# algoterranean/3dgan

Hardware: AMD Instinct MI355X
Metric: images/sec (whole node), CIFAR-10 IWGAN bs=512 (higher is better)
Workload: dtype bf16; 1 GPU; --model iwgan --dataset cifar(32x32x3 synthetic) --batch_size 512/GPU --latent_size 200 --optimizer adam --lr 1e-4 --beta1 0.5 --beta2 0.9 --n_disc_train 5; one step = 5 D + 1 G optimizer steps on 6 fresh batches; global_batch=512, parallelism=dp1, ranks_seen=1

## Files before the change

3dgan_amd/csrc/tdg_igemm.hip:

```cpp
#include <stdlib.h>

#include "tdg_igemm.h"
#include "tdg_wgrad_patch.h"
#include <type_traits>

#define OOB_OFFSET 0xFFFFFF00u

#ifdef TDG_STAMPS
#define TDG_STAMP(var)                                                                            \
  do {                                                                                            \
    __builtin_amdgcn_sched_barrier(0);                                                            \
    asm volatile("s_memtime %0\n\ts_waitcnt lgkmcnt(0)" : "=s"(var)::"memory");                  \
    __builtin_amdgcn_sched_barrier(0);                                                            \
  } while (0)
#else
#define TDG_STAMP(var) do { } while (0)
#endif

template <int I, int N, class F>
__device__ __forceinline__ void static_for(F&& f) {
  if constexpr (I < N) {
    f(IntC<I>{});
    static_for<I + 1, N>(f);
  }
// ... 965 lines not shown
    if (mmode != TDG_MASK_NONE) {
#pragma unroll
      for (int e = 0; e < 8; ++e) v[e] = (bf16_t)((float)v[e] * ((float)mv[it][e] > 0.f ? 1.f : mlow));
      if (args.col_partial) *reinterpret_cast<bf16x8*>(sE + row * PE + cc * 16) = v;
    }
    if (n + 8 <= N) {
      *reinterpret_cast<bf16x8*>(out + p + n) = v;
    } else {
      *reinterpret_cast<bf16x4*>(out + p + n) = bf16x4{v[0], v[1], v[2], v[3]};
    }
  }
  if (args.col_partial) {
    constexpr int G = NTHR / BN > 0 ? NTHR / BN : 1;
    float* sRed = reinterpret_cast<float*>(smem + BM * PE + BM * 8);
    __syncthreads();
    const int mlim = args.col_images > 0 ? min(M, args.col_images * cl.GH * cl.GW * (cl.nbh * cl.nbw > 1 ? cl.nbh * cl.nbw : 1)) : M;
    const int rows_valid = max(0, min(BM, mlim - m0));
    const int col = tid % BN, grp = tid / BN;
    const bool bnm = args.col_mode == TDG_COL_BN;
    if (grp < G) {
      const float piv = bnm ? sBias[col] : 0.f;
      float s0 = 0.f, s1 = 0.f;
      for (int r = grp; r < rows_valid; r += G) {
        const float v = (float)*reinterpret_cast<const bf16_t*>(sE + r * PE + col * 2) - piv;
        s0 += v;
        s1 += v * v;
      }
      sRed[(grp * 2 + 0) * BN + col] = s0;
      sRed[(grp * 2 + 1) * BN + col] = s1;
    }
    __syncthreads();
    if (tid < BN && n0 + tid < N) {
      float t0 = 0.f, t1 = 0.f;
#pragma unroll
      for (int g = 0; g < G; ++g) { t0 += sRed[(g * 2 + 0) * BN + tid]; t1 += sRed[(g * 2 + 1) * BN + tid]; }
      float* pr = args.col_partial + (size_t)(blockIdx.z * args.ntiles_m_max + tile_m) * 2 * N;
      pr[n0 + tid] = t0;
      pr[N + n0 + tid] = t1;
    }
  }
}

#ifndef PT_VBLOCK
#define PT_VBLOCK 32
#endif
#ifndef PT_LA
#define PT_LA 3
#endif
template <int TM, int TN, int ABL, int t>
__device__ __forceinline__ void patch_half0(f32x4 (&acc)[TM][TN], const bf16x8 (&fa0)[TM], bf16x8 (&fa1)[TM], bf16x8 (&fb)[2 * TN + PT_LA],
                                            const char* smem, const int (&a1)[TM], const char* pB, int coff0, int coff1) {
  if constexpr (t < TN) {
    constexpr int t2 = t + PT_LA, ks2 = t2 / TN, j2 = t2 - ks2 * TN;
    if constexpr (ABL != 1) fb[t2] = *reinterpret_cast<const bf16x8*>(pB + j2 * 16 * IG_BKB + (ks2 ? coff1 : coff0));
    else fb[t2] = fb[t2 & 1];
    if constexpr (t < TM && ABL != 2) fa1[t] = pt_lds_frag(a1[t]);
#pragma unroll
    for (int i = 0; i < TM; ++i) Mma<bf16_t>::run(acc[i][t], fb[t], fa0[i]);
    __builtin_amdgcn_sched_group_barrier(0x100, 1 + (t < TM ? 1 : 0), 0);
    __builtin_amdgcn_sched_group_barrier(0x008, TM, 0);
    patch_half0<TM, TN, ABL, t + 1>(acc, fa0, fa1, fb, smem, a1, pB, coff0, coff1);
  }
}
template <int TM, int TN, int ABL, int t>
__device__ __forceinline__ void patch_half1(f32x4 (&acc)[TM][TN], bf16x8 (&fa0)[TM], const bf16x8 (&fa1)[TM], bf16x8 (&fb)[2 * TN + PT_LA],
                                            const char* smem, const int (&a0n)[TM], const char* pB, const char* pBn, int coff0, int coff1) {
  constexpr int NT = 2 * TN;
  if constexpr (t < NT) {
    constexpr int j = t - TN, t2 = t + PT_LA;
    if constexpr (ABL == 1) fb[t2] = fb[t2 & 1];
    else if constexpr (t2 < NT) fb[t2] = *reinterpret_cast<const bf16x8*>(pB + (t2 - TN) * 16 * IG_BKB + coff1);
    else fb[t2] = *reinterpret_cast<const bf16x8*>(pBn + (t2 - NT) * 16 * IG_BKB + coff0);
    constexpr int a_lo = TN > TM ? (j >= 1 && j <= TM ? j - 1 : 0) : (j * TM) / TN;
    constexpr int a_hi = TN > TM ? (j >= 1 && j <= TM ? j : 0) : ((j + 1) * TM) / TN;
    if constexpr (ABL != 2) static_for<a_lo, a_hi>([&](auto i_c) { constexpr int i = decltype(i_c)::value; fa0[i] = pt_lds_frag(a0n[i]); });
#pragma unroll
    for (int i = 0; i < TM; ++i) Mma<bf16_t>::run(acc[i][j], fb[t], fa1[i]);
    __builtin_amdgcn_sched_group_barrier(0x100, 1 + (a_hi - a_lo), 0);
    __builtin_amdgcn_sched_group_barrier(0x008, TM, 0);
    patch_half1<TM, TN, ABL, t + 1>(acc, fa0, fa1, fb, smem, a0n, pB, pBn, coff0, coff1);
  }
}

template <int BM, int BN, int ABL, int CK = PT_CK, int PIECES = PT_PIECES>
__global__ void __launch_bounds__(512, 2) igemm_fwd_patch_kernel(const IgArgs args) {
  using T = bf16_t;
  constexpr int NTHR = 512, CW = 4, LW = 4;
  constexpr int PATCHB = PIECES * 1024, PPW = (PIECES + LW - 1) / LW, PPW0 = (PPW + 1) / 2;
  constexpr int WMR = BM / CW, TM = WMR / 16, TN = BN / 16;
  constexpr int BNL = 2 * ((BN / 16 + 1) / 2) * 16;
  constexpr int NIB = BNL / 8, NBJ = (NIB + LW - 1) / LW;
  constexpr int STAGE = BNL * IG_BKB, NS = 3;
  static_assert(PIECES % LW == 0, "patch pieces are dealt evenly to the loader waves");
  static_assert(BM % (16 * CW) == 0 && BN % 16 == 0 && BN / 16 >= BM / (16 * CW), "tile config: the K step hands out one A fragment per column tile");
  constexpr int OFF_ZERO = 0, OFF_RING = PT_ZEROB, OFF_PATCH = OFF_RING + NS * STAGE, OFF_TAB = OFF_PATCH + PT_NPB * PATCHB;
  typedef __attribute__((address_space(3))) void* lds_ptr_t;

  extern __shared__ __attribute__((aligned(16))) char smem[];
  const IgClass& cl = args.cls[blockIdx.z];
  const int tid = threadIdx.x;
  const int bid = xcd_remap(blockIdx.x, gridDim.x);
  const int tile_m = bid / args.ntiles_n;
  const int tile_n = bid - tile_m * args.ntiles_n;
  const int M = cl.M;
  const int nsteps = cl.nsteps;
  int* sTab = reinterpret_cast<int*>(smem + OFF_TAB);
  float* sBias = reinterpret_cast<float*>(smem + OFF_TAB + nsteps * 8 * 8);
  if (tile_m * BM >= M) {
    if (args.col_partial && tid < BN) {
      const int n = args.n_begin + tile_n * BN + tid;
      float* pr = args.col_partial + (size_t)(blockIdx.z * args.ntiles_m_max + tile_m) * 2 * args.N;
      if (n < args.N) { pr[n] = 0.f; pr[args.N + n] = 0.f; }
    }
    return;
  }
  const int m0 = tile_m * BM, n0 = args.n_begin + tile_n * BN;
  const int wave = __builtin_amdgcn_readfirstlane(tid >> 6), lane = tid & 63;
  const bool is_mma = wave < CW;
  const int ntaps = cl.ntaps, G = cl.ngroups, QH = cl.QH, QW = cl.QW;
  const int GHW = cl.GH * cl.GW;
  const int SLC = ntaps * CK;
  const int halo = cl.halo;
  const int P = args.nslices * G;

  unsigned long long ph0 = 0, ph1 = 0, php = 0, t0 = 0, t1 = 0, t2 = 0, s_issue = 0, s_mma = 0, s_sync = 0;
  unsigned long long q0 = 0, q1 = 0, q2 = 0, q3 = 0;
  TDG_STAMP(ph0);
  const float bias_v = (tid < BNL && args.bias && n0 + tid < args.N) ? args.bias[n0 + tid] : 0.f;
  if (tid < PT_ZEROB / 4) reinterpret_cast<int*>(smem + OFF_ZERO)[tid] = 0;
  if ((unsigned)(size_t)(lds_ptr_t)smem != 0u) __builtin_trap();
  TDG_STAMP(q0);
  int tapvec = 0;
  if (is_mma) {
    int tw[IG_MAX_TAPS / 2], g_t0[4], g_ph[4], g_pw[4];
    const int sgs = args.sigma - 1;
#pragma unroll
    for (int k = 0; k < IG_MAX_TAPS / 2; ++k) tw[k] = reinterpret_cast<const int*>(cl.tap)[k];
#pragma unroll
    for (int k = 0; k < 4; ++k) { g_t0[k] = cl.grp[k].t0; g_ph[k] = cl.grp[k].ph; g_pw[k] = cl.grp[k].pw; }
    {
      const int t = lane & (IG_MAX_TAPS - 1);
      int w = tw[0];
#pragma unroll
      for (int k = 1; k < IG_MAX_TAPS / 2; ++k) w = (t >> 1) == k ? tw[k] : w;
      int gi = 0, ph = g_ph[0], pw = g_pw[0];
#pragma unroll
      for (int k = 1; k < 4; ++k) {
        const bool in = k < G && t >= g_t0[k];
        gi = in ? k : gi; ph = in ? g_ph[k] : ph; pw = in ? g_pw[k] : pw;
      }
      const int pk = (t & 1) ? (w >> 16) : w;
      const int dhq = (tap_dh(pk) - ph) >> sgs, dwq = (tap_dw(pk) - pw) >> sgs;
      tapvec = gi | ((dhq + 8) << 4) | ((dwq + 8) << 8);
    }
    TDG_STAMP(q1);
    for (int g0 = 0; g0 < nsteps * 8; g0 += 64 * CW) {
      const int g = g0 + tid;
      const unsigned u = fd_div((unsigned)g, args.fd_ck);
      const int j = g - (int)u * CK;
      const unsigned sl = fd_div(u, cl.fd_nt);
      const int t = (int)(u - sl * (unsigned)ntaps);
      const int tv = __builtin_amdgcn_ds_bpermute((t & 31) << 2, tapvec);
      int w0 = 0, w1 = 31;
      if ((int)sl < args.nslices) {
        const int gi = tv & 15, dhq = ((tv >> 4) & 15) - 8, dwq = ((tv >> 8) & 15) - 8;
        const int p = (int)sl * G + gi;
        const int buf = p - (p / PT_NPB) * PT_NPB;
        w0 = OFF_PATCH + buf * PATCHB + (dhq * QW + dwq) * PT_PIXB + j * 16;
        w1 = t;
      }
      if (g < nsteps * 8) {
        sTab[2 * g] = w0;
        sTab[2 * g + 1] = w1;
      }
    }
// ... 3 lines not shown
  TDG_STAMP(q3);

  const int r16 = lane & 15, q = lane >> 4;
  f32x4 acc[TM][TN];
#pragma unroll
  for (int i = 0; i < TM; ++i)
#pragma unroll
    for (int j = 0; j < TN; ++j) acc[i][j] = f32x4{0.f, 0.f, 0.f, 0.f};

  if (!is_mma) {
    const int lwave = wave - CW;
    const int par = lwave & 1, wh = lwave >> 1, rsub = lane >> 3;
    const __amdgpu_buffer_rsrc_t rA = make_rsrc(args.src, args.src_bytes);
    const __amdgpu_buffer_rsrc_t rB = make_rsrc(static_cast<const char*>(args.wpack) + cl.w_off_bytes, args.w_bytes - cl.w_off_bytes);
    const int lch = (lane & 7) ^ ((4 * par + (rsub >> 1)) & 7);
    unsigned b_row[NBJ];
    int b_lds[NBJ];
#pragma unroll
    for (int j = 0; j < NBJ; ++j) {
      const int I = 2 * (wh + (LW / 2) * j) + par;
      const int n = n0 + 8 * I + rsub;
      const bool useful = 8 * I < BN;
      b_row[j] = (useful && n < args.N) ? ((unsigned)n * (unsigned)cl.Kp + (unsigned)(lch * 8)) * 2u : OOB_OFFSET;
      b_lds[j] = (I < NIB ? I : NIB - 1) * 1024;
    }
    auto b_pieces = [&](int step) {
      const int st = step - (step / NS) * NS;
      char* stage = smem + OFF_RING + st * STAGE;
      const unsigned kb = step < nsteps ? (unsigned)step * IG_BKB : OOB_OFFSET;
#pragma unroll
      for (int j = 0; j < NBJ; ++j) {
        const unsigned off = (b_row[j] == OOB_OFFSET || kb == OOB_OFFSET) ? OOB_OFFSET : b_row[j] + kb;
        __builtin_amdgcn_raw_ptr_buffer_load_lds(rB, (lds_ptr_t)(stage + b_lds[j]), 16, off, 0, 0, 0);
      }
    };
    struct Ph { int sl, gi, buf; };
    auto ph_next = [&](Ph& x) {
      if (++x.gi == G) { x.gi = 0; ++x.sl; }
      x.buf = x.buf == PT_NPB - 1 ? 0 : x.buf + 1;
    };
    auto ph_end_chunk = [&](const Ph& x) { return x.sl * SLC + (cl.grp[x.gi].t0 + cl.grp[x.gi].nt) * CK; };
    auto ph_delta = [&](const Ph& x) { return (unsigned)(((cl.grp[x.gi].ph * args.SW + cl.grp[x.gi].pw) * args.Cs + x.sl * CK * 8) * 2); };
    asm volatile("s_waitcnt lgkmcnt(0)" ::: "memory");
    b_pieces(0);
    const int IPT = BM / GHW;
    const int nimg = M / GHW;
    const int nblk = cl.nbh * cl.nbw;
    const int LH = args.SH / args.sigma, LW_ = args.SW / args.sigma;
    unsigned a_src[PPW];
#pragma unroll
    for (int ps = 0; ps < PPW; ++ps) {
      const int c = (ps * LW + lwave) * 64 + lane;
      const int pl = c / PT_CK, j = c - pl * PT_CK;
      const unsigned il = fd_div((unsigned)pl, cl.fd_qhw);
      const int rem = pl - (int)il * QH * QW;
      const int qh = (int)fd_div((unsigned)rem, cl.fd_qw), qw = rem - qh * QW;
      const int blk = tile_m * IPT + (int)il;
      bool ok = (int)il < IPT && blk < nimg && j < CK;
      int img = blk, lh = qh, lw = qw;
      if (nblk > 1) {
        img = blk / nblk;
        const int br = blk - img * nblk, bi = br / cl.nbw, bj = br - bi * cl.nbw;
        lh = bi * cl.GH - halo + qh;
        lw = bj * cl.GW - halo + qw;
        ok = ok && (unsigned)lh < (unsigned)LH && (unsigned)lw < (unsigned)LW_;
      }
      a_src[ps] = ok ? (unsigned)((((img * args.SH + args.sigma * lh) * args.SW + args.sigma * lw) * args.Cs + j * 8) * 2) : OOB_OFFSET;
    }
    auto a_piece = [&](const Ph& x, unsigned delta, auto ps_c) {
      constexpr int ps = decltype(ps_c)::value;
      const unsigned off = a_src[ps] == OOB_OFFSET ? OOB_OFFSET : a_src[ps] + delta;
      __builtin_amdgcn_raw_ptr_buffer_load_lds(rA, (lds_ptr_t)(smem + OFF_PATCH + x.buf * PATCHB + (ps * LW + lwave) * 1024), 16, off, 0, 0, 0);
    };
    auto a_pieces = [&](const Ph& x, unsigned delta, auto lo_c, auto hi_c) {
      static_for<decltype(lo_c)::value, decltype(hi_c)::value>([&](auto ps_c) { a_piece(x, delta, ps_c); });
    };
    Ph pn{0, 0, 0};
    {
      const unsigned dl0 = ph_delta(pn);
      a_pieces(pn, dl0, IntC<0>{}, IntC<PPW>{});
      ph_next(pn);
    }
    b_pieces(1);
    TDG_STAMP(t0);
    s_mma = t0 - ph0;
    asm volatile("s_waitcnt vmcnt(%0)" ::"n"(NBJ) : "memory");
    __builtin_amdgcn_s_barrier();
    TDG_STAMP(php);
    Ph pf{0, 0, 0};
    int left = P - 1;
    int ready = P > PT_NPB ? (ph_end_chunk(pf) - 1) / 8 + 1 : (1 << 30);
    if (ready < PT_NPB - 1) ready = PT_NPB - 1;
    unsigned dl = left > 0 ? ph_delta(pn) : 0u;
    asm volatile("s_waitcnt vmcnt(0)" ::: "memory");
    for (int step = 0; step < nsteps; ++step) {
      TDG_STAMP(t0);
      __builtin_amdgcn_s_barrier();
      TDG_STAMP(t1);
      if constexpr (ABL != 4) b_pieces(step + 2);
      if constexpr (ABL == 4) {
      } else if (step < PT_NPB - 1) {
        if (left > 0) {
          a_pieces(pn, dl, IntC<0>{}, IntC<PPW>{});
          ph_next(pn);
          --left;
          dl = left > 0 ? ph_delta(pn) : 0u;
        }
      } else if (step == ready) {
        a_pieces(pn, dl, IntC<0>{}, IntC<PPW0>{});
      } else if (step == ready + 1) {
        a_pieces(pn, dl, IntC<PPW0>{}, IntC<PPW>{});
        ph_next(pn);
        ph_next(pf);
        --left;
        ready = left > 0 ? max((ph_end_chunk(pf) - 1) / 8 + 1, step + 1) : (1 << 30);
        dl = left > 0 ? ph_delta(pn) : 0u;
      }
      TDG_STAMP(t2);
      asm volatile("s_waitcnt vmcnt(0)" ::: "memory");
      s_sync += t1 - t0; s_issue += t2 - t1;
    }
    __builtin_amdgcn_s_barrier();
  } else {
    int base_i[TM], mask_i[TM];
    {
      int a_i[TM], b_i[TM];
      unsigned rowbits[TM], colbits[TM];
      bool ok_i[TM];
#pragma unroll
      for (int i = 0; i < TM; ++i) {
        const int loc = wave * WMR + i * 16 + r16;
        ok_i[i] = m0 + loc < M;
        const unsigned il = fd_div((unsigned)loc, cl.fd_ghw);
        const int rem = loc - (int)il * GHW;
        a_i[i] = (int)fd_div((unsigned)rem, cl.fd_gw);
        b_i[i] = rem - a_i[i] * cl.GW;
        base_i[i] = (((int)il * QH + a_i[i] + halo) * QW + b_i[i] + halo) * PT_PIXB;
        rowbits[i] = colbits[i] = 0u;
      }
      const bool is_tap = lane < 32 && lane < ntaps;
      const int my_dh = ((tapvec >> 4) & 15) - 8, my_dw = ((tapvec >> 8) & 15) - 8;
      for (int d = -8; d < 8; ++d) {
        const unsigned tr = (unsigned)__builtin_amdgcn_ballot_w64(is_tap && my_dh == d);
        const unsigned tc = (unsigned)__builtin_amdgcn_ballot_w64(is_tap && my_dw == d);
        if (tr | tc) {
#pragma unroll
          for (int i = 0; i < TM; ++i) {
            rowbits[i] |= (unsigned)(a_i[i] + halo + d) < (unsigned)QH ? tr : 0u;
            colbits[i] |= (unsigned)(b_i[i] + halo + d) < (unsigned)QW ? tc : 0u;
          }
        }
      }
#pragma unroll
      for (int i = 0; i < TM; ++i) mask_i[i] = ok_i[i] ? (int)(rowbits[i] & colbits[i]) : 0;
    }
    const int swl = (r16 >> 1) & 7;
    const int coff0 = ((0 * 4 + q) ^ swl) << 4, coff1 = ((1 * 4 + q) ^ swl) << 4;
    auto a_offsets = [&](const i32x2& e, int (&o)[TM]) {
#pragma unroll
      for (int i = 0; i < TM; ++i) o[i] = (base_i[i] + e[0]) & __builtin_amdgcn_sbfe(mask_i[i], e[1], 1);
    };
    const i32x2* sTab2 = reinterpret_cast<const i32x2*>(sTab);
    asm volatile("s_waitcnt lgkmcnt(0)" ::: "memory");
    TDG_STAMP(t0);
    s_issue = t0 - ph0;
    __builtin_amdgcn_s_barrier();
    TDG_STAMP(php);
    int a0[TM], a1[TM];
    a_offsets(sTab2[q], a0);
    a_offsets(sTab2[4 + q], a1);
    i32x2 e0 = sTab2[(nsteps > 1 ? 8 : 0) + q], e1 = sTab2[(nsteps > 1 ? 8 : 0) + 4 + q];
    bf16x8 fa0[TM], fa1[TM];
    bf16x8 fb[2 * TN + PT_LA];
    {
      const char* pB = smem + OFF_RING + r16 * IG_BKB;
#pragma unroll
      for (int i = 0; i < TM; ++i) fa0[i] = pt_lds_frag(a0[i]);
#pragma unroll
      for (int k = 0; k < PT_LA; ++k) fb[k] = *reinterpret_cast<const bf16x8*>(pB + k * 16 * IG_BKB + coff0);
    }
    int st = 0;
    for (int step = 0; step < nsteps; ++step) {
      TDG_STAMP(t0);
      const int stn = st == NS - 1 ? 0 : st + 1;
      const char* pB = smem + OFF_RING + st * STAGE + r16 * IG_BKB;
      const char* pBn = smem + OFF_RING + stn * STAGE + r16 * IG_BKB;
      int a0n[TM], a1n[TM];
      if constexpr (ABL == 3) {
#pragma unroll
        for (int i = 0; i < TM; ++i) { a0n[i] = a0[i]; a1n[i] = a1[i]; }
      } else {
        a_offsets(e0, a0n);
        a_offsets(e1, a1n);
      }
      const int s2 = step + 2 < nsteps ? step + 2 : step;
      e0 = sTab2[s2 * 8 + q];
      e1 = sTab2[s2 * 8 + 4 + q];
      __builtin_amdgcn_sched_group_barrier(0x002, PT_VBLOCK, 0);
      __builtin_amdgcn_sched_group_barrier(0x100, 1, 0);
      patch_half0<TM, TN, ABL, 0>(acc, fa0, fa1, fb, smem, a1, pB, coff0, coff1);
      TDG_STAMP(t1);
      __builtin_amdgcn_s_barrier();
      TDG_STAMP(t2);
      patch_half1<TM, TN, ABL, TN>(acc, fa0, fa1, fb, smem, a0n, pB, pBn, coff0, coff1);
#pragma unroll
      for (int k = 0; k < PT_LA; ++k) fb[k] = fb[2 * TN + k];
#pragma unroll
      for (int i = 0; i < TM; ++i) a1[i] = a1n[i];
      st = stn;
      s_sync += t2 - t1;
    }
    asm volatile("s_waitcnt lgkmcnt(0)" ::: "memory");
    __builtin_amdgcn_s_barrier();
  }
  TDG_STAMP(ph1);
#ifdef TDG_STAMPS
  if (args.stamps && lane == 0) {
    unsigned long long* o = args.stamps + ((size_t)(blockIdx.z * gridDim.x + blockIdx.x) * 8 + wave) * 4;
    o[0] = s_issue; o[1] = s_mma; o[2] = s_sync; o[3] = (unsigned long long)nsteps;
  }
#endif

  static_assert(BM * (BN * 2 + 16) + BM * 8 + 2 * (NTHR / BN) * BN * 4 <= OFF_TAB, "epilogue staging must not reach the tables");
  staged_epilogue_bf16<BM, BN, TM, TN, NTHR>(acc, smem, sBias, is_mma, wave * WMR, 0, TN, tid, r16, q, m0, n0, M, tile_m, args, cl);
#ifdef TDG_STAMPS
  if (args.stamps) {
    unsigned long long ph3 = 0;
    asm volatile("s_waitcnt vmcnt(0)" ::: "memory");
    TDG_STAMP(ph3);
    if (lane == 0) {
      unsigned long long* o = args.stamps + 262144 + ((size_t)(blockIdx.z * gridDim.x + blockIdx.x) * 8 + wave) * 4;
      o[0] = ph0; o[1] = php; o[2] = ph1; o[3] = ph3;
      unsigned long long* o2 = args.stamps + 524288 + ((size_t)(blockIdx.z * gridDim.x + blockIdx.x) * 8 + wave) * 4;
      o2[0] = q0 - ph0; o2[1] = q1 - ph0; o2[2] = q2 - ph0; o2[3] = q3 - ph0;
    }
  }
#endif
}

__device__ __forceinline__ void bp_dma(const i32x4& rsrc, unsigned voff, unsigned soff, unsigned lds_byte) {
  asm volatile("s_mov_b32 m0, %3\n\ts_nop 0\n\tbuffer_load_dwordx4 %0, %1, %2 offen lds" ::"v"(voff), "s"(rsrc), "s"(soff), "s"(lds_byte) : "memory");
}
#define BP_PIECES 28
#define BP_NSLOT(BN) (((BN) / 8 + BP_PIECES / 2 + 7) / 8)
#define BP_NTAIL(BN) ((BN) / 32 - ((BN) / 64 > 0 ? (BN) / 64 : 1))
#define BP_NPB(BN) (BP_NSLOT(BN) / 2 < BP_NTAIL(BN) ? BP_NSLOT(BN) / 2 : BP_NTAIL(BN))
template <int BN>
__global__ void __launch_bounds__(512, 2) igemm_fwd_bp_kernel(const IgArgs args) {
  using T = bf16_t;
  constexpr int BM = 256, NTHR = 512, TM = 4, TN = BN / 32;
  constexpr int STAGE = BN * IG_BKB, NS = 3, PATCHB = BP_PIECES * 1024;
  constexpr int NBP = BN / 8;
  constexpr int NPH = BP_PIECES / 2;
  constexpr int NSLOT = (NBP + NPH + 7) / 8;
  constexpr int OFF_RING = PT_ZEROB, OFF_PATCH = OFF_RING + NS * STAGE, OFF_DUMMY = OFF_PATCH + PT_NPB * PATCHB, OFF_TAB = OFF_DUMMY + 1024;
  typedef __attribute__((address_space(3))) void* lds_ptr_t;
  extern __shared__ __attribute__((aligned(16))) char smem[];
  const IgClass& cl = args.cls[blockIdx.z];
  const int tid = threadIdx.x;
  const int bid = xcd_remap(blockIdx.x, gridDim.x);
  const int tile_m = bid / args.ntiles_n;
  const int tile_n = bid - tile_m * args.ntiles_n;
  const int M = cl.M, nsteps = cl.nsteps, ntaps = cl.ntaps, G = cl.ngroups, QW = cl.QW, QH = cl.QH, halo = cl.halo;
  const unsigned lds0 = (unsigned)(size_t)(lds_ptr_t)smem;
  int* sU = reinterpret_cast<int*>(smem + OFF_TAB);
  float* sBias = reinterpret_cast<float*>(smem + OFF_TAB + 2 * nsteps * 4);
  if (tile_m * BM >= M) {
    if (args.col_partial && tid < BN) {
      const int n = args.n_begin + tile_n * BN + tid;
      float* pr = args.col_partial + (size_t)(blockIdx.z * args.ntiles_m_max + tile_m) * 2 * args.N;
      if (n < args.N) { pr[n] = 0.f; pr[args.N + n] = 0.f; }
    }
    return;
  }
  const int m0 = tile_m * BM, n0 = args.n_begin + tile_n * BN;
  const int wave = __builtin_amdgcn_readfirstlane(tid >> 6), lane = tid & 63;
  const int wm = wave & 3, wn = wave >> 2;
  const int r16 = lane & 15, q = lane >> 4;
  const int sgs = args.sigma - 1;

  unsigned long long bs0 = 0, bs1 = 0, bs2 = 0, bs3 = 0, bw_wait = 0, bw_bar = 0;
  TDG_STAMP(bs0);
  if (tid < PT_ZEROB / 4) reinterpret_cast<int*>(smem)[tid] = 0;
  for (int u = tid; u < 2 * nsteps; u += NTHR) {
    const unsigned sl = fd_div((unsigned)u, cl.fd_nt);
    const int t = u - (int)sl * ntaps;
    int gi = 0;
#pragma unroll
    for (int k = 1; k < 4; ++k) gi = (k < G && t >= cl.grp[k].t0) ? k : gi;
    const int pk = cl.tap[t];
    const int dhq = (tap_dh(pk) - cl.grp[gi].ph) >> sgs, dwq = (tap_dw(pk) - cl.grp[gi].pw) >> sgs;
    const int ph = (int)sl * G + gi;
    sU[u] = (int)lds0 + OFF_PATCH + (ph % PT_NPB) * PATCHB + (dhq * QW + dwq) * PT_PIXB;
// ... 1499 lines not shown
}

namespace {

inline int pick_bn(int n) {
  if (n <= 16) return 16;
  if (n <= 64) return 64;
  const double w128 = (double)tdg_round_up(n, 128) / n, w208 = (double)tdg_round_up(n, 208) / n;
  return w208 < w128 - 1e-9 ? 208 : 128;
}

#ifdef TDG_STAMPS
inline unsigned long long* stamp_ptr() {
  return getenv("TDG_STAMP_PTR") ? (unsigned long long*)strtoull(getenv("TDG_STAMP_PTR"), nullptr, 0) : nullptr;
}
#endif

void grant_col_partial(IgArgs& a, const TdgEpilogue* epi) {
  if (!epi || !epi->col_partial || epi->col_mode == TDG_COL_NONE || !epi->col_nblk_out) return;
  const int nblk = a.nclasses * a.ntiles_m_max;
  if ((size_t)nblk * 2 * a.N * sizeof(float) > epi->col_partial_bytes) return;
  a.col_partial = epi->col_partial;
  a.col_mode = epi->col_mode;
  a.col_images = epi->col_images;
  *epi->col_nblk_out = nblk;
}

template <typename T, int BM, int BN, int WGM, int WGN>
int launch_fwd_cfg(const IgArgs& a, bool veca, int grid_x, double flops, hipStream_t s) {
  const size_t lds = (size_t)(BM + BN) * IG_BKB + IG_MAX_TAPS * sizeof(int);
  const dim3 grid(grid_x, 1, a.nclasses), block(256);
  const char* name = TDG_NAME("igemm_fwd_kernel<%s,%d,%d>", sizeof(T) == 2 ? "bf16" : "f32", BM, BN);
  return tdg_launch(name, 0, flops, s, [&] {
    if (veca)
      hipLaunchKernelGGL((igemm_fwd_kernel<T, BM, BN, WGM, WGN, true>), grid, block, lds, s, a);
    else
      hipLaunchKernelGGL((igemm_fwd_kernel<T, BM, BN, WGM, WGN, false>), grid, block, lds, s, a);
  });
}

template <typename T, int BM, int BN, int NS, int NW = 8, int WS = 0>
int launch_fwd_dma(IgArgs& a, int mmax, double flops, const TdgEpilogue* epi, hipStream_t s) {
  a.n_begin = 0;
  a.ntiles_n = tdg_ceil_div(a.N, BN);
  a.ntiles_m_max = tdg_ceil_div(mmax, BM);
  if (sizeof(T) == 2 && !a.accumulate && (a.N & 3) == 0) grant_col_partial(a, epi);
  constexpr int BNL = 2 * ((BN / 16 + 1) / 2) * 16;
  const size_t lds = NS * (size_t)(BM + BNL) * IG_BKB + IG_MAX_TAPS * sizeof(int) + BNL * sizeof(float);
  static_assert(NS * (size_t)(BM + BNL) * IG_BKB + IG_MAX_TAPS * sizeof(int) + BNL * sizeof(float) <= 160 * 1024, "LDS budget");
  a.slab_rows = a.ntiles_m_max * BM;
  int smax = 0;
  for (int c = 0; c < a.nclasses; ++c) smax = a.cls[c].nsteps > smax ? a.cls[c].nsteps : smax;
  const long long wgs = (long long)a.ntiles_n * a.ntiles_m_max * a.nclasses;
  const int ks_force = getenv("TDG_KSPLIT") ? atoi(getenv("TDG_KSPLIT")) : 0;
  if (!WS && epi && epi->splitk_ws && epi->splitk_ws_bytes && wgs <= 128 && smax >= 16 && ks_force != 1) {
    int want = (int)(256 / wgs);
    if (want > smax / 4) want = smax / 4;
    if (want > 8) want = 8;
    if (ks_force > 1) want = ks_force;
    const int per = tdg_ceil_div(smax, want);
    const int nsplit = tdg_ceil_div(smax, per);
    const size_t need = (size_t)nsplit * a.nclasses * a.slab_rows * a.N * sizeof(float);
    if (nsplit > 1 && need <= epi->splitk_ws_bytes) {
      a.ksplit = nsplit;
      a.steps_per_split = per;
      a.slab = static_cast<float*>(epi->splitk_ws);
      a.col_partial = nullptr;
      if (epi->col_nblk_out) *epi->col_nblk_out = 0;
    }
  }
  const dim3 grid(a.ntiles_n * a.ntiles_m_max, a.ksplit, a.nclasses), block(64 * NW);
  const char* name = TDG_NAME(WS ? "igemm_fwd_dma_kernel<%s,%d,%d,%d,8,1>" : (NW == 8 ? "igemm_fwd_dma_kernel<%s,%d,%d,%d>" : "igemm_fwd_dma_kernel<%s,%d,%d,%d,4,0>"), sizeof(T) == 2 ? "bf16" : "f32", BM, BN, NS);
  return tdg_launch<igemm_fwd_dma_kernel<T, BM, BN, NS, NW, WS>>(name, (int)lds, flops, s, [&] {
    hipLaunchKernelGGL((igemm_fwd_dma_kernel<T, BM, BN, NS, NW, WS>), grid, block, lds, s, a);
    if (a.ksplit > 1) {
      int mmx = 0;
      for (int c = 0; c < a.nclasses; ++c) mmx = a.cls[c].M > mmx ? a.cls[c].M : mmx;
      const long long items = (long long)mmx * ((a.N + 3) / 4);
      hipLaunchKernelGGL((splitk_finish_kernel<T>), dim3((unsigned)((items + 255) / 256), 1, a.nclasses), dim3(256), 0, s, a);
    }
  });
}

template <int BM, int BN = 208, int CK = PT_CK, int PIECES = PT_PIECES, bool FORCE_HALO = false>
bool plan_fwd_patch(IgArgs& a, int mmax) {
  const int enabled = getenv("TDG_PATCH") ? atoi(getenv("TDG_PATCH")) : 1;
  if (!enabled || (int)a.fd_ck.d != CK || a.accumulate || (a.N & 3) || (a.Cso & 3)) return false;
  if (a.sigma < 1 || a.sigma > 2 || a.SH % a.sigma || a.SW % a.sigma) return false;
  const int LH = a.SH / a.sigma, LWd = a.SW / a.sigma;
  if (enabled != 2 && (long long)tdg_ceil_div(mmax, BM) * tdg_ceil_div(a.N, BN) * a.nclasses < 160) return false;
  struct Geo { int bh, bw, nbh, nbw, halo, QH, QW; } geo[IG_MAX_CLASSES];
  for (int ci = 0; ci < a.nclasses; ++ci) {
    IgClass& c = a.cls[ci];
    if (c.nbh * c.nbw > 1) return false;
    const int ghw = c.GH * c.GW;
    if (ghw <= 0 || c.M % ghw) return false;
    if (c.nsteps < 4 || c.nsteps * 64 > 16384 || c.ntaps > 31) return false;
    int ng = 0, dmax = 0;
    for (int t = 0; t < c.ntaps; ++t) {
      const int dh = (signed char)(c.tap[t] & 0xff), dw = (signed char)((c.tap[t] >> 8) & 0xff);
      const int ph = ((dh % a.sigma) + a.sigma) % a.sigma, pw = ((dw % a.sigma) + a.sigma) % a.sigma;
      const int dhq = (dh - ph) / a.sigma, dwq = (dw - pw) / a.sigma;
      if (dhq < -8 || dhq > 7 || dwq < -8 || dwq > 7) return false;
      dmax = abs(dhq) > dmax ? abs(dhq) : dmax;
      dmax = abs(dwq) > dmax ? abs(dwq) : dmax;
      if (ng && c.grp[ng - 1].ph == ph && c.grp[ng - 1].pw == pw) { ++c.grp[ng - 1].nt; continue; }
      for (int g = 0; g < ng; ++g)
        if (c.grp[g].ph == ph && c.grp[g].pw == pw) return false;
      if (ng == 4) return false;
      c.grp[ng].t0 = t; c.grp[ng].nt = 1; c.grp[ng].ph = ph; c.grp[ng].pw = pw;
      ++ng;
    }
    c.ngroups = ng;
    Geo& g = geo[ci];
    if (BM % ghw == 0 && !(FORCE_HALO && ghw == BM)) {
      g = Geo{c.GH, c.GW, 1, 1, 0, LH, LWd};
    } else {
      int bw = c.GW < 16 ? c.GW : 16;
      while (bw > 1 && (c.GW % bw || BM % bw)) --bw;
      const int bh = BM / bw;
      if (bh * bw != BM || c.GH % bh || c.GW % bw) return false;
      g = Geo{bh, bw, c.GH / bh, c.GW / bw, dmax, bh + 2 * dmax, bw + 2 * dmax};
    }
    if (g.QW > 32 || g.QH > 64) return false;
    if ((BM / (g.bh * g.bw)) * g.QH * g.QW * PT_PIXB > PIECES * 1024 || g.bh > g.QH + 8 || g.bw > g.QW + 8) return false;
    for (int t = 0; t < c.ntaps; ++t) {
      const int dh = (signed char)(c.tap[t] & 0xff), dw = (signed char)((c.tap[t] >> 8) & 0xff);
      const int ph = ((dh % a.sigma) + a.sigma) % a.sigma, pw = ((dw % a.sigma) + a.sigma) % a.sigma;
      const int off = ((dh - ph) / a.sigma) * g.QW + (dw - pw) / a.sigma;
      if (off < -127 || off > 127) return false;
    }
    const int P = a.nslices * ng, slc = c.ntaps * CK;
    auto first_chunk = [&](int p) { return (p / ng) * slc + c.grp[p % ng].t0 * CK; };
    auto end_chunk = [&](int p) { return (p / ng) * slc + (c.grp[p % ng].t0 + c.grp[p % ng].nt) * CK; };
    for (int p = 1; p < PT_NPB && p < P; ++p)
      if (first_chunk(p) / 8 < (p - 1) + 2) return false;
    int prev_issue = PT_NPB - 3;
    for (int p = PT_NPB; p < P; ++p) {
      const int ready = (end_chunk(p - PT_NPB) - 1) / 8 + 1;
      const int issue = ready > prev_issue + 2 ? ready : prev_issue + 2;
      if (first_chunk(p) / 8 < issue + 3) return false;
      prev_issue = issue;
    }
  }
  for (int ci = 0; ci < a.nclasses; ++ci) {
    IgClass& c = a.cls[ci];
    const Geo& g = geo[ci];
    c.QH = g.QH; c.QW = g.QW;
    c.fd_qhw = make_fastdiv(g.QH * g.QW); c.fd_qw = make_fastdiv(g.QW);
    c.nbh = g.nbh; c.nbw = g.nbw; c.halo = g.halo;
    if (g.nbh * g.nbw > 1) {
      c.GH = g.bh; c.GW = g.bw;
      c.fd_ghw = make_fastdiv(g.bh * g.bw); c.fd_gw = make_fastdiv(g.bw);
    }
  }
  return true;
}

template <int BM, int BN, int CK = PT_CK, int PIECES = PT_PIECES>
int launch_fwd_patch(IgArgs& a, int mmax, double flops, const TdgEpilogue* epi, hipStream_t s) {
  a.n_begin = 0;
  a.ntiles_n = tdg_ceil_div(a.N, BN);
  a.ntiles_m_max = tdg_ceil_div(mmax, BM);
  grant_col_partial(a, epi);
  int smax = 0;
  for (int c = 0; c < a.nclasses; ++c) smax = a.cls[c].nsteps > smax ? a.cls[c].nsteps : smax;
  constexpr int BNL = 2 * ((BN / 16 + 1) / 2) * 16;
  const size_t lds = PT_ZEROB + 3 * (size_t)BNL * IG_BKB + PT_NPB * (size_t)PIECES * 1024 + (size_t)smax * 64 + BNL * sizeof(float);
  if (lds > 160 * 1024) {
    tdg_set_error("igemm_fwd_patch: %zu bytes of LDS", lds);
    return TDG_EUNSUPPORTED;
  }
  const dim3 grid(a.ntiles_n * a.ntiles_m_max, 1, a.nclasses), block(512);
  const char* name = TDG_NAME("igemm_fwd_patch_kernel<bf16,%d,%d>", BM, BN);
  auto go = [&](auto abl) {
    constexpr int ABL = decltype(abl)::value;
    return tdg_launch<igemm_fwd_patch_kernel<BM, BN, ABL, CK, PIECES>>(name, 160 * 1024, flops, s, [&] {
      hipLaunchKernelGGL((igemm_fwd_patch_kernel<BM, BN, ABL, CK, PIECES>), grid, block, lds, s, a);
    });
  };
#ifdef TDG_STAMPS
  if constexpr (BM == 192) {
    const int abl = getenv("TDG_PATCH_ABL") ? atoi(getenv("TDG_PATCH_ABL")) : 0;
    if (abl == 1) return go(IntC<1>{});
    if (abl == 2) return go(IntC<2>{});
    if (abl == 3) return go(IntC<3>{});
    if (abl == 4) return go(IntC<4>{});
  }
#endif
  return go(IntC<0>{});
}

template <int BN>
bool plan_fwd_bp(IgArgs& a, int mmax) {
  const char* e = getenv("TDG_BP");
  if (e && atoi(e) == 0) return false;
  IgArgs t = a;
  if (!plan_fwd_patch<256, BN, 4, BP_PIECES, true>(t, mmax)) return false;
  for (int ci = 0; ci < t.nclasses; ++ci) {
    const IgClass& c = t.cls[ci];
    if (c.GH * c.GW != 256 || c.halo < 1 || c.QH * c.QW * PT_PIXB > BP_PIECES * 1024) return false;
    if (c.ntaps % 4 || c.ntaps != 4 * c.ngroups) return false;
    for (int g = 0; g < c.ngroups; ++g)
      if (c.grp[g].nt != 4) return false;
    if (c.nsteps != 2 * t.nslices * c.ngroups || c.M % 256) return false;
  }
  a = t;
  return true;
}

template <int BN>
int launch_fwd_bp(IgArgs& a, int mmax, double flops, const TdgEpilogue* epi, hipStream_t s) {
  a.n_begin = 0;
  a.ntiles_n = tdg_ceil_div(a.N, BN);
  a.ntiles_m_max = tdg_ceil_div(mmax, 256);
  grant_col_partial(a, epi);
  int smax = 0;
  for (int c = 0; c < a.nclasses; ++c) smax = a.cls[c].nsteps > smax ? a.cls[c].nsteps : smax;
  const size_t lds = PT_ZEROB + 3 * (size_t)BN * IG_BKB + PT_NPB * (size_t)BP_PIECES * 1024 + 1024 + (size_t)smax * 8 + BN * sizeof(float);
  if (lds > 160 * 1024) {
    tdg_set_error("igemm_fwd_bp: %zu bytes of LDS", lds);
    return TDG_EUNSUPPORTED;
  }
#ifdef TDG_STAMPS
  a.stamps = stamp_ptr();
#endif
  const dim3 grid(a.ntiles_n * a.ntiles_m_max, 1, a.nclasses), block(512);
  return tdg_launch<igemm_fwd_bp_kernel<BN>>(TDG_NAME("igemm_fwd_bp_kernel<bf16,256,%d>", BN), 160 * 1024, flops, s, [&] {
    hipLaunchKernelGGL((igemm_fwd_bp_kernel<BN>), grid, block, lds, s, a);
  });
}

template <typename T>
int launch_fwd(IgArgs& a, bool veca, int bn, double flops, const TdgEpilogue* epi, hipStream_t s) {
  constexpr int BM = 128;
#ifdef TDG_STAMPS
  static const int dbg = getenv("TDG_DEBUG_ABLATE") ? atoi(getenv("TDG_DEBUG_ABLATE")) : 0;
#else
  const int dbg = 0;
#endif
  const char* dma_env = getenv("TDG_DMA");
  const int dma_mode = dma_env ? atoi(dma_env) : 1;
  a.debug = dbg;
#ifdef TDG_STAMPS
  a.stamps = stamp_ptr();
#endif
  int mmax = 0;
  for (int c = 0; c < a.nclasses; ++c) mmax = a.cls[c].M > mmax ? a.cls[c].M : mmax;
  if constexpr (sizeof(T) == 2) {
    if (veca && bn == 208 && dma_mode == 1 && !getenv("TDG_DMA_BM") && !getenv("TDG_DMA_NW")) {
      const long long per = (long long)tdg_ceil_div(a.N, 208) * a.nclasses;
      const double c192 = (double)tdg_ceil_div(per * tdg_ceil_div(mmax, 192), 256) * 192 / 1.0;
      const double c128 = (double)tdg_ceil_div(per * tdg_ceil_div(mmax, 128), 256) * 128 / 0.75;
      const int pbm = getenv("TDG_PATCH_BM") ? atoi(getenv("TDG_PATCH_BM")) : 0;
      const bool want128 = pbm ? pbm == 128 : c128 < c192 - 1e-9;
      if (want128 && plan_fwd_patch<128>(a, mmax)) return launch_fwd_patch<128, 208>(a, mmax, flops, epi, s);
      if (plan_fwd_patch<192>(a, mmax)) return launch_fwd_patch<192, 208>(a, mmax, flops, epi, s);
      if (!want128 && !pbm && plan_fwd_patch<128>(a, mmax)) return launch_fwd_patch<128, 208>(a, mmax, flops, epi, s);
    }
  }
  if (veca && bn == 208 && dma_mode && (a.N & 3) == 0 && (a.Cso & 3) == 0) {
    const long long per = (long long)tdg_ceil_div(a.N, 208) * a.nclasses;
    static const int force = getenv("TDG_DMA_BM") ? atoi(getenv("TDG_DMA_BM")) : 0;
    const int bms[3] = {256, 192, 128};
    double eff[3] = {0.72, 1.0, 0.83};
    if (const char* e = getenv("TDG_EFF")) sscanf(e, "%lf,%lf,%lf", &eff[0], &eff[1], &eff[2]);
    int best = 0;
    double best_cost = 1e30;
    for (int i = 0; i < 3; ++i) {
      const long long tiles = per * tdg_ceil_div(mmax, bms[i]);
      const double cost = (double)tdg_ceil_div(tiles, 256) * bms[i] / eff[i];
      if (cost < best_cost - 1e-9) { best_cost = cost; best = i; }
    }
    int bm = force ? force : bms[best];
    if (dma_mode == 3) bm = 192;
    if (dma_mode == 4) bm = 256;
    static const int ring192 = getenv("TDG_RING") ? atoi(getenv("TDG_RING")) : 3;
    if (bm == 128) {
      const char* n112_env = getenv("TDG_FWD_N112");
      if (per * tdg_ceil_div(mmax, 128) <= 128 && a.N > 112 && !(n112_env && atoi(n112_env) == 0)) {
        const long long wg112 = (long long)tdg_ceil_div(a.N, 112) * a.nclasses * tdg_ceil_div(mmax, 128);
        if (wg112 <= 128 && !(n112_env && atoi(n112_env) == 1)) return launch_fwd_dma<T, 64, 112, 3>(a, mmax, flops, epi, s);
        return launch_fwd_dma<T, 128, 112, 3>(a, mmax, flops, epi, s);
      }
      if constexpr (sizeof(T) == 2) {
        const char* nw_env = getenv("TDG_DMA_NW");
        const char* ws128_env = getenv("TDG_WS128");
        if (!a.accumulate && !(nw_env && atoi(nw_env) != 44) && !(ws128_env && atoi(ws128_env) == 0))
          return launch_fwd_dma<T, 128, 208, 3, 8, 1>(a, mmax, flops, epi, s);
      }
      return launch_fwd_dma<T, 128, 208, 3>(a, mmax, flops, epi, s);
    }
    const char* nw_env = getenv("TDG_DMA_NW");
    const int nw192 = nw_env ? atoi(nw_env) : 44;
    if constexpr (sizeof(T) == 2)
      if (bm == 192 && nw192 == 44 && !a.accumulate && ring192 != 2) return launch_fwd_dma<T, 192, 208, 3, 8, 1>(a, mmax, flops, epi, s);
    if (bm == 192) return ring192 == 2 ? launch_fwd_dma<T, 192, 208, 2>(a, mmax, flops, epi, s) : launch_fwd_dma<T, 192, 208, 3>(a, mmax, flops, epi, s);
    return launch_fwd_dma<T, 256, 208, 2>(a, mmax, flops, epi, s);
  }
  if constexpr (sizeof(T) == 2) {
    if (veca && dma_mode == 1 && (bn == 128 || bn == 64) && !getenv("TDG_DMA_BM") && !getenv("TDG_DMA_NW")) {
      if (bn == 128 && a.N > 112 && plan_fwd_bp<128>(a, mmax)) return launch_fwd_bp<128>(a, mmax, flops, epi, s);
      if (bn == 64 && a.N > 32 && plan_fwd_bp<64>(a, mmax)) return launch_fwd_bp<64>(a, mmax, flops, epi, s);
      if (bn == 128 && a.N > 112 && plan_fwd_patch<256, 128, 4, 28>(a, mmax)) return launch_fwd_patch<256, 128, 4, 28>(a, mmax, flops, epi, s);
      if (bn == 64 && a.N > 32 && plan_fwd_patch<256, 64, 4, 28>(a, mmax)) return launch_fwd_patch<256, 64, 4, 28>(a, mmax, flops, epi, s);
    }
  }
  if (veca && bn == 128 && dma_mode && (a.N & 3) == 0 && (a.Cso & 3) == 0) {
    const int bnt = a.N <= 112 ? 112 : 128;
    const long long per = (long long)tdg_ceil_div(a.N, bnt) * a.nclasses;
    const long long t256 = per * tdg_ceil_div(mmax, 256), t128 = per * tdg_ceil_div(mmax, 128);
    const double c256 = (double)tdg_ceil_div(t256, 256) * 256, c128 = (double)tdg_ceil_div(t128, 256) * 128 / 0.85;
    if (bnt == 112) return c128 < c256 ? launch_fwd_dma<T, 128, 112, 3>(a, mmax, flops, epi, s) : launch_fwd_dma<T, 256, 112, 3>(a, mmax, flops, epi, s);
    return c128 < c256 ? launch_fwd_dma<T, 128, 128, 3>(a, mmax, flops, epi, s) : launch_fwd_dma<T, 256, 128, 3>(a, mmax, flops, epi, s);
  }
  if (veca && bn == 64 && dma_mode && (a.N & 3) == 0 && (a.Cso & 3) == 0 && a.N > 32) return launch_fwd_dma<T, 128, 64, 3>(a, mmax, flops, epi, s);
  a.ntiles_n = tdg_ceil_div(a.N, bn);
  a.ntiles_m_max = tdg_ceil_div(mmax, BM);
  int gx = a.ntiles_n * a.ntiles_m_max;
  if (bn == 208 && (long long)gx * a.nclasses < 384) {
    a.ntiles_m_max = tdg_ceil_div(mmax, 64);
    gx = a.ntiles_n * a.ntiles_m_max;
    return launch_fwd_cfg<T, 64, 208, 4, 1>(a, veca, gx, flops, s);
  }
  switch (bn) {
    case 16: return launch_fwd_cfg<T, BM, 16, 4, 1>(a, veca, gx, flops, s);
    case 64: return launch_fwd_cfg<T, BM, 64, 4, 1>(a, veca, gx, flops, s);
    case 128: return launch_fwd_cfg<T, BM, 128, 2, 2>(a, veca, gx, flops, s);
    case 208: return launch_fwd_cfg<T, BM, 208, 4, 1>(a, veca, gx, flops, s);
  }
  tdg_set_error("igemm_fwd: no tile config for BN=%d", bn);
  return TDG_EUNSUPPORTED;
}

template <typename T, int BKK, int BN, int WGK, int WGN>
int launch_wgrad_cfg(const WgArgs& a, bool veca, double flops, hipStream_t s) {
  constexpr int MR = WgGeom<T>::MR;
  const size_t lds = (size_t)MR * (WgGeom<T>::pitch(BKK) + WgGeom<T>::pitch(BN)) + IG_MAX_TAPS * sizeof(int);
  const dim3 grid(a.ntiles_k * a.ntiles_n, 1, a.nsplit), block(256);
  const char* name = TDG_NAME("igemm_wgrad_kernel<%s,%d,%d>", sizeof(T) == 2 ? "bf16" : "f32", BKK, BN);
  return tdg_launch(name, 0, flops, s, [&] {
// ... 954 lines not shown
```

Baseline: 30830 images/sec.

## Add 4-stage B ring with lagged loader waits for BM=128 patch conv kernel

Adds an NS template parameter to the forward patch implicit-GEMM kernel. With NS=4 the loader waves issue B and patch loads one step further ahead and wait only on the older batch, using per-step vmcnt counts, instead of draining all outstanding loads each step. A new BM=128 launch path prefers a 12-piece patch with the 4-stage ring when it fits in LDS and the plan check passes with the extra lag, falling back to the older variants otherwise. The BM=128 versus 192 selection efficiency factor is also nudged. Costs are more LDS per block and stricter planning constraints.

```diff
diff --git a/3dgan_amd/csrc/tdg_igemm.hip b/3dgan_amd/csrc/tdg_igemm.hip
--- a/3dgan_amd/csrc/tdg_igemm.hip
+++ b/3dgan_amd/csrc/tdg_igemm.hip
@@ -1071,7 +1071,7 @@
   }
 }
 
-template <int BM, int BN, int ABL, int CK = PT_CK, int PIECES = PT_PIECES>
+template <int BM, int BN, int ABL, int CK = PT_CK, int PIECES = PT_PIECES, int NS = 3>
 __global__ void __launch_bounds__(512, 2) igemm_fwd_patch_kernel(const IgArgs args) {
   using T = bf16_t;
   constexpr int NTHR = 512, CW = 4, LW = 4;
@@ -1079,7 +1079,8 @@
   constexpr int WMR = BM / CW, TM = WMR / 16, TN = BN / 16;
   constexpr int BNL = 2 * ((BN / 16 + 1) / 2) * 16;
   constexpr int NIB = BNL / 8, NBJ = (NIB + LW - 1) / LW;
-  constexpr int STAGE = BNL * IG_BKB, NS = 3;
+  constexpr int STAGE = BNL * IG_BKB, LAG = NS - 3;
+  static_assert(NS == 3 || NS == 4, "3-stage ring, or 4 stages with the loaders' wait one step behind their issue");
   static_assert(PIECES % LW == 0, "patch pieces are dealt evenly to the loader waves");
   static_assert(BM % (16 * CW) == 0 && BN % 16 == 0 && BN / 16 >= BM / (16 * CW), "tile config: the K step hands out one A fragment per column tile");
   constexpr int OFF_ZERO = 0, OFF_RING = PT_ZEROB, OFF_PATCH = OFF_RING + NS * STAGE, OFF_TAB = OFF_PATCH + PT_NPB * PATCHB;
@@ -1249,32 +1250,58 @@
       ph_next(pn);
     }
     b_pieces(1);
+    int left = P - 1;
+    unsigned dl = left > 0 ? ph_delta(pn) : 0u;
+    bool early1 = false;
+    if constexpr (LAG) {
+      b_pieces(2);
+      if (left > 0) {
+        a_pieces(pn, dl, IntC<0>{}, IntC<PPW>{});
+        ph_next(pn);
+        --left;
+        dl = left > 0 ? ph_delta(pn) : 0u;
+        early1 = true;
+      }
+    }
     TDG_STAMP(t0);
     s_mma = t0 - ph0;
-    asm volatile("s_waitcnt vmcnt(%0)" ::"n"(NBJ) : "memory");
+    if constexpr (!LAG) {
+      asm volatile("s_waitcnt vmcnt(%0)" ::"n"(NBJ) : "memory");
+    } else if (early1) {
+      asm volatile("s_waitcnt vmcnt(%0)" ::"n"(2 * NBJ + PPW) : "memory");
+    } else {
+      asm volatile("s_waitcnt vmcnt(%0)" ::"n"(2 * NBJ) : "memory");
+    }
     __builtin_amdgcn_s_barrier();
     TDG_STAMP(php);
     Ph pf{0, 0, 0};
-    int left = P - 1;
     int ready = P > PT_NPB ? (ph_end_chunk(pf) - 1) / 8 + 1 : (1 << 30);
     if (ready < PT_NPB - 1) ready = PT_NPB - 1;
-    unsigned dl = left > 0 ? ph_delta(pn) : 0u;
-    asm volatile("s_waitcnt vmcnt(0)" ::: "memory");
+    if constexpr (!LAG) {
+      asm volatile("s_waitcnt vmcnt(0)" ::: "memory");
+    } else if (early1) {
+      asm volatile("s_waitcnt vmcnt(%0)" ::"n"(NBJ + PPW) : "memory");
+    } else {
+      asm volatile("s_waitcnt vmcnt(%0)" ::"n"(NBJ) : "memory");
+    }
     for (int step = 0; step < nsteps; ++step) {
       TDG_STAMP(t0);
       __builtin_amdgcn_s_barrier();
       TDG_STAMP(t1);
-      if constexpr (ABL != 4) b_pieces(step + 2);
+      if constexpr (ABL != 4) b_pieces(step + NS - 1);
+      int mine = 0;
       if constexpr (ABL == 4) {
-      } else if (step < PT_NPB - 1) {
+      } else if (step < PT_NPB - 1 - LAG) {
         if (left > 0) {
           a_pieces(pn, dl, IntC<0>{}, IntC<PPW>{});
           ph_next(pn);
           --left;
           dl = left > 0 ? ph_delta(pn) : 0u;
+          mine = PPW;
         }
       } else if (step == ready) {
         a_pieces(pn, dl, IntC<0>{}, IntC<PPW0>{});
+        mine = PPW0;
       } else if (step == ready + 1) {
         a_pieces(pn, dl, IntC<PPW0>{}, IntC<PPW>{});
         ph_next(pn);
@@ -1282,11 +1309,20 @@
         --left;
         ready = left > 0 ? max((ph_end_chunk(pf) - 1) / 8 + 1, step + 1) : (1 << 30);
         dl = left > 0 ? ph_delta(pn) : 0u;
+        mine = PPW - PPW0;
       }
       TDG_STAMP(t2);
-      asm volatile("s_waitcnt vmcnt(0)" ::: "memory");
+      if constexpr (!LAG) {
+        asm volatile("s_waitcnt vmcnt(0)" ::: "memory");
+      } else {
+        if (mine == 0) asm volatile("s_waitcnt vmcnt(%0)" ::"n"(NBJ) : "memory");
+        else if (mine == PPW - PPW0) asm volatile("s_waitcnt vmcnt(%0)" ::"n"(NBJ + PPW - PPW0) : "memory");
+        else if (mine == PPW0) asm volatile("s_waitcnt vmcnt(%0)" ::"n"(NBJ + PPW0) : "memory");
+        else asm volatile("s_waitcnt vmcnt(%0)" ::"n"(NBJ + PPW) : "memory");
+      }
       s_sync += t1 - t0; s_issue += t2 - t1;
     }
+    if constexpr (LAG) asm volatile("s_waitcnt vmcnt(0)" ::: "memory");
     __builtin_amdgcn_s_barrier();
   } else {
     int base_i[TM], mask_i[TM];
@@ -1375,7 +1411,7 @@
 #pragma unroll
       for (int i = 0; i < TM; ++i) a1[i] = a1n[i];
       st = stn;
-      s_sync += t2 - t1;
+      s_sync += t2 - t1; s_mma += t1 - t0;
     }
     asm volatile("s_waitcnt lgkmcnt(0)" ::: "memory");
     __builtin_amdgcn_s_barrier();
@@ -3041,7 +3077,7 @@
   });
 }
 
-template <int BM, int BN = 208, int CK = PT_CK, int PIECES = PT_PIECES, bool FORCE_HALO = false>
+template <int BM, int BN = 208, int CK = PT_CK, int PIECES = PT_PIECES, bool FORCE_HALO = false, int LAG = 0>
 bool plan_fwd_patch(IgArgs& a, int mmax) {
   const int enabled = getenv("TDG_PATCH") ? atoi(getenv("TDG_PATCH")) : 1;
   if (!enabled || (int)a.fd_ck.d != CK || a.accumulate || (a.N & 3) || (a.Cso & 3)) return false;
@@ -3098,7 +3134,7 @@
     for (int p = PT_NPB; p < P; ++p) {
       const int ready = (end_chunk(p - PT_NPB) - 1) / 8 + 1;
       const int issue = ready > prev_issue + 2 ? ready : prev_issue + 2;
-      if (first_chunk(p) / 8 < issue + 3) return false;
+      if (first_chunk(p) / 8 < issue + 3 + LAG) return false;
       prev_issue = issue;
     }
   }
@@ -3116,26 +3152,32 @@
   return true;
 }
 
-template <int BM, int BN, int CK = PT_CK, int PIECES = PT_PIECES>
+template <int BN, int PIECES, int NS>
+size_t fwd_patch_lds(const IgArgs& a) {
+  int smax = 0;
+  for (int c = 0; c < a.nclasses; ++c) smax = a.cls[c].nsteps > smax ? a.cls[c].nsteps : smax;
+  constexpr int BNL = 2 * ((BN / 16 + 1) / 2) * 16;
+  return PT_ZEROB + NS * (size_t)BNL * IG_BKB + PT_NPB * (size_t)PIECES * 1024 + (size_t)smax * 64 + BNL * sizeof(float);
+}
+
+template <int BM, int BN, int CK = PT_CK, int PIECES = PT_PIECES, int NS = 3>
 int launch_fwd_patch(IgArgs& a, int mmax, double flops, const TdgEpilogue* epi, hipStream_t s) {
   a.n_begin = 0;
   a.ntiles_n = tdg_ceil_div(a.N, BN);
   a.ntiles_m_max = tdg_ceil_div(mmax, BM);
   grant_col_partial(a, epi);
-  int smax = 0;
-  for (int c = 0; c < a.nclasses; ++c) smax = a.cls[c].nsteps > smax ? a.cls[c].nsteps : smax;
-  constexpr int BNL = 2 * ((BN / 16 + 1) / 2) * 16;
-  const size_t lds = PT_ZEROB + 3 * (size_t)BNL * IG_BKB + PT_NPB * (size_t)PIECES * 1024 + (size_t)smax * 64 + BNL * sizeof(float);
+  const size_t lds = fwd_patch_lds<BN, PIECES, NS>(a);
   if (lds > 160 * 1024) {
     tdg_set_error("igemm_fwd_patch: %zu bytes of LDS", lds);
     return TDG_EUNSUPPORTED;
   }
   const dim3 grid(a.ntiles_n * a.ntiles_m_max, 1, a.nclasses), block(512);
-  const char* name = TDG_NAME("igemm_fwd_patch_kernel<bf16,%d,%d>", BM, BN);
+  const char* name = BM == 128 && BN == 208 && (PIECES != 12 || NS != 4) ? TDG_NAME("igemm_fwd_patch_kernel<bf16,%d,%d,%d,%d>", BM, BN, PIECES, NS)
+                                                                       : TDG_NAME("igemm_fwd_patch_kernel<bf16,%d,%d>", BM, BN);
   auto go = [&](auto abl) {
     constexpr int ABL = decltype(abl)::value;
-    return tdg_launch<igemm_fwd_patch_kernel<BM, BN, ABL, CK, PIECES>>(name, 160 * 1024, flops, s, [&] {
-      hipLaunchKernelGGL((igemm_fwd_patch_kernel<BM, BN, ABL, CK, PIECES>), grid, block, lds, s, a);
+    return tdg_launch<igemm_fwd_patch_kernel<BM, BN, ABL, CK, PIECES, NS>>(name, 160 * 1024, flops, s, [&] {
+      hipLaunchKernelGGL((igemm_fwd_patch_kernel<BM, BN, ABL, CK, PIECES, NS>), grid, block, lds, s, a);
     });
   };
 #ifdef TDG_STAMPS
@@ -3148,6 +3190,20 @@
   }
 #endif
   return go(IntC<0>{});
+}
+
+inline bool launch_fwd_patch128(IgArgs& a, int mmax, double flops, const TdgEpilogue* epi, hipStream_t s, int* rc) {
+  const int form = getenv("TDG_PATCH128") ? atoi(getenv("TDG_PATCH128")) : 2;
+  constexpr int P128 = 12;
+  if (form >= 2 && fwd_patch_lds<208, P128, 4>(a) <= 160 * 1024 && plan_fwd_patch<128, 208, PT_CK, P128, false, 1>(a, mmax))
+    *rc = launch_fwd_patch<128, 208, PT_CK, P128, 4>(a, mmax, flops, epi, s);
+  else if (form >= 1 && plan_fwd_patch<128, 208, PT_CK, P128>(a, mmax))
+    *rc = launch_fwd_patch<128, 208, PT_CK, P128>(a, mmax, flops, epi, s);
+  else if (plan_fwd_patch<128>(a, mmax))
+    *rc = launch_fwd_patch<128, 208>(a, mmax, flops, epi, s);
+  else
+    return false;
+  return true;
 }
 
 template <int BN>
@@ -3210,12 +3266,13 @@
     if (veca && bn == 208 && dma_mode == 1 && !getenv("TDG_DMA_BM") && !getenv("TDG_DMA_NW")) {
       const long long per = (long long)tdg_ceil_div(a.N, 208) * a.nclasses;
       const double c192 = (double)tdg_ceil_div(per * tdg_ceil_div(mmax, 192), 256) * 192 / 1.0;
-      const double c128 = (double)tdg_ceil_div(per * tdg_ceil_div(mmax, 128), 256) * 128 / 0.75;
+      const double c128 = (double)tdg_ceil_div(per * tdg_ceil_div(mmax, 128), 256) * 128 / 0.78;
       const int pbm = getenv("TDG_PATCH_BM") ? atoi(getenv("TDG_PATCH_BM")) : 0;
       const bool want128 = pbm ? pbm == 128 : c128 < c192 - 1e-9;
-      if (want128 && plan_fwd_patch<128>(a, mmax)) return launch_fwd_patch<128, 208>(a, mmax, flops, epi, s);
+      int rc = TDG_OK;
+      if (want128 && launch_fwd_patch128(a, mmax, flops, epi, s, &rc)) return rc;
       if (plan_fwd_patch<192>(a, mmax)) return launch_fwd_patch<192, 208>(a, mmax, flops, epi, s);
-      if (!want128 && !pbm && plan_fwd_patch<128>(a, mmax)) return launch_fwd_patch<128, 208>(a, mmax, flops, epi, s);
+      if (!want128 && !pbm && launch_fwd_patch128(a, mmax, flops, epi, s, &rc)) return rc;
     }
   }
   if (veca && bn == 208 && dma_mode && (a.N & 3) == 0 && (a.Cso & 3) == 0) {
```

After: 31280 images/sec, median of 6. +1.5%, better.
